# Levicoz/Options-model

Measured on AMD Instinct MI355X. Metric: paths x steps / sec (whole American pricing: path-gen + LSM + mean), higher is better.
Workload: dtype f32

## Files before the change

### options_model_amd/csrc/omc_api.hip

```cpp
#include <sched.h>

#include <algorithm>

#include "omc_ctx.h"

namespace omc::abi {

thread_local std::string g_err;
size_t g_alloc_limit = 0;

int check_market(double S0, double K, double T, double r)
{
    if (!(S0 > 0) || !(K > 0) || !(T > 0)) return fail(-1, "S0, K, T must be positive.");
    if (!(r >= 0)) return fail(-2, "r must be non-negative.");
    return 0;
}

int check_sizes(int64_t n_paths, int n_steps)
{
    if (n_paths <= 0 || n_steps <= 0)
        return fail(-3, "num_simulations and num_time_steps must be positive integers.");
    if (n_steps > omc::kMaxSteps) return fail(-8, "num_time_steps exceeds the supported maximum (4094).");
    return 0;
}
// ... 689 lines not shown
    int rc = bind_in(c);
    if (rc) return rc;
    if (!bytes) return 0;
    HIP_TRY(hipMemcpyAsync(dst, src, bytes, kind, c->stream));
    HIP_TRY(hipStreamSynchronize(c->stream));
    return 0;
}

int omc_memcpy_h2d(omc_ctx* c, void* dst, const void* src, size_t bytes)
{
    return copy_and_wait(c, dst, src, bytes, hipMemcpyHostToDevice);
}

int omc_memcpy_d2h(omc_ctx* c, void* dst, const void* src, size_t bytes)
{
    return copy_and_wait(c, dst, src, bytes, hipMemcpyDeviceToHost);
}

int omc_set_option(omc_ctx* c, const char* key, int64_t value)
{
    if (!c || !key) return fail(-7, "null pointer.");
    if (!strcmp(key, "gbm_vec")) c->gbm_vec = (int)value;
    else if (!strcmp(key, "alloc_limit")) g_alloc_limit = value > 0 ? (size_t)value : 0;
    else if (!strcmp(key, "fold_antithetic")) c->fold = value <= 0 ? 0 : (value >= 2 ? 2 : 1);
    else if (!strcmp(key, "pass2_tables")) c->pass2_tables = value ? 1 : 0;
    else if (!strcmp(key, "pass2_tables_irregular_every")) c->pass2_irr_every = value > 0 ? (int)value : 0;
    else if (!strcmp(key, "heston_vec")) c->heston_vec = (int)value;
    else if (!strcmp(key, "world_size")) c->world = value > 0 ? (int)value : 1;
    else if (!strcmp(key, "step_graph")) c->step_graph = value < 0 ? -1 : (value ? 1 : 0);
    else if (!strcmp(key, "seq_overlap")) c->seq_overlap = value < 0 ? -1 : (value ? 1 : 0);
    else if (!strcmp(key, "seq_event_stride")) c->seq_event_stride = value > 0 ? (int)value : 0;
    else if (!strcmp(key, "seq_step_k")) c->seq_step_k = value < 0 ? -1 : (int)(value > 32 ? 32 : value);
    else if (!strcmp(key, "seq_two_pass_k")) c->seq_two_pass_k = value < 0 ? -1 : (int)(value > 32 ? 32 : value);
    else if (!strcmp(key, "bounds_exercise_every")) {
        if (value < 0 || value > 2147483647) return fail(-4, "bounds_exercise_every must be in 0 .. 2^31 - 1.");
        c->bounds_every = value;
    }
    else if (!strcmp(key, "bounds_control_variate")) {
        if (value != 0 && value != 1) return fail(-4, "bounds_control_variate must be 0 or 1.");
        c->bounds_cv = (int)value;
    }
    else if (!strcmp(key, "bounds_cv_form")) {
        if (value != 0 && value != 1) return fail(-4, "bounds_cv_form must be 0 or 1.");
        c->bounds_cv_form = (int)value;
    }
    else if (!strcmp(key, "chain_fused")) c->chain_fused = value ? 1 : 0;
    else if (!strcmp(key, "chain_k")) c->chain_k = value < 1 ? -1 : (int)(value > 16 ? 16 : value);
    else if (!strcmp(key, "seq_step_wgs")) c->seq_step_wgs = value > 0 ? (int)value : 0;
    else if (!strcmp(key, "p2p_exchange")) c->p2p_use = value ? 1 : 0;
    else if (!strcmp(key, "p2p_deadline_ms") || !strcmp(key, "p2p_first_deadline_ms")) {
        if (value <= 0) return fail(-4, "a p2p deadline must be positive.");
        (key[4] == 'f' ? c->p2p_first_deadline_s : c->p2p_deadline_s) = (double)value * 1e-3;
        if (c->p2p) omc::p2p_set_deadline(c->p2p, c->p2p_deadline_s, c->p2p_first_deadline_s);
    }
    else return fail(-4, "unknown option key.");
    return 0;
}

int omc_set_allreduce_hook(omc_ctx* c, omc_allreduce_fn fn, void* user)
{
    if (!c) return fail(-7, "null context.");
    if (fn) {
        int rc;
        if ((rc = bind(c))) return rc;
        if ((rc = c->seq_vote.ensure(kVoteBytes))) return rc;
    }
// ... 128 lines not shown
```

### options_model_amd/csrc/omc_api_seq.hip

```cpp
#include <cstdlib>

#include "omc_ctx.h"

using namespace omc::abi;

extern "C" {

static int pricing_events(omc_ctx* c, int i, hipEvent_t** out)
{
    const int k = c->seq_event_stride, s = i == 0 ? 0 : (k > 0 && i % k == 0) ? i / k : -1;
    *out = s == 0 ? c->ev : nullptr;
    if (s <= 0) return 0;
    while (c->ev_pool.size() < 7 * (size_t)s) {
        hipEvent_t e = nullptr;
        HIP_TRY(hipEventCreate(&e));
        c->ev_pool.push_back(e);
    }
    *out = c->ev_pool.data() + 7 * (size_t)(s - 1);
    return 0;
}

static bool seq_overlap_enabled(const omc_ctx* c)
{
    if (c->seq_overlap >= 0) return c->seq_overlap != 0;
// ... 248 lines not shown
        }
        if (i0 == 0 && p2p) omc::p2p_begin_call(c->p2p);
        if (i0 == 0) HIP_TRY(hipEventRecord(c->ev[0], c->stream));
        for (int k = 0; k < Kb; ++k)
            if ((rc = enqueue_paths(c, &p[i0 + k], (float*)((char*)c->mS.p + sbytes * (size_t)k), ld))) return rc;
        if (i0 == 0) HIP_TRY(hipEventRecord(c->ev[1], c->stream));
        for (int t = N; t >= 1; --t) {
            HIP_TRY(omc::lsm_step_multi(c->stream, c->mtable.p, Kb, G, sem, vec4, N, t));
            if (ext && t >= 2) {
                if (p2p) {
                    HIP_TRY(omc::p2p_exchange_step_multi(c->p2p, c->stream, Kb, t - 1));
                    c->p2p_used = true;
                } else {
                    HIP_TRY(omc::lsm_reduce_step_moments_multi(c->stream, c->mtable.p, Kb, t - 1));
                    if ((rc = allreduce(c, gmomK + (size_t)(t - 1) * 8 * (size_t)Kb, 8 * Kb))) return rc;
                }
            }
        }
        HIP_TRY(omc::lsm_final_multi(c->stream, c->mtable.p, Kb, M));
        if (i0 == 0) HIP_TRY(hipEventRecord(c->ev[2], c->stream));
    }
    return 0;
}

int omc_seq_step_width(omc_ctx* c, const omc_params* p, int n)
{
    if (!c || !p || n <= 0) return 0;
    for (int i = 0; i < n; ++i)
        if (check_params(&p[i])) return 0;
    return seq_multi_width(c, p, n);
}


static bool seq_group_eligible(const omc_ctx* c, const omc_params* q)
{
    return c->pass2_tables && q->semantics == OMC_SEM_TWO_PASS && q->n_steps >= 2 && fold_applies(c, q);
}

static int seq_group_run(const omc_ctx* c, const omc_params* p, int n)
{
    if (c->distributed() || !seq_group_eligible(c, &p[0])) return 1;
    double c0, g;
    omc::gbm_fold_constants(p[0].S0, p[0].K, p[0].r, p[0].sigma, p[0].T, p[0].n_steps, &c0, &g);
    int run = 1;
    for (; run < n; ++run) {
        const omc_params& q = p[run];
        if (!seq_group_eligible(c, &q) || q.n_paths != p[0].n_paths || q.n_steps != p[0].n_steps || q.r != p[0].r ||
            q.T != p[0].T)
            break;
        double c0q, gq;
        omc::gbm_fold_constants(q.S0, q.K, q.r, q.sigma, q.T, q.n_steps, &c0q, &gq);
        if (c0q != c0 || gq != g) break;
    }
    return run;
}

static size_t seq_group_matrix_bytes(const omc_params* p)
{
    return sizeof(float) * (size_t)padded_ld(p->n_paths / 2) * ((size_t)p->n_steps + 1);
}

static int seq_group_ideal(const omc_ctx* c, const omc_params* p, int run)
{
    if (run < 2) return 1;
    static const int env_k = getenv("OMC_SEQ_TWO_PASS_K") ? atoi(getenv("OMC_SEQ_TWO_PASS_K")) : -1;
    int k = c->seq_two_pass_k >= 0 ? c->seq_two_pass_k : env_k;
    if (k < 0) k = (double)p[0].n_paths * (double)p[0].n_steps > 536870912.0 ? 1 : 8;
    if (k > omc::kSeqGroupMax) k = omc::kSeqGroupMax;
    if (k > run) k = run;
    return k < 2 ? 1 : k;
}

static int seq_group_fit(const omc_ctx* c, const omc_params* p, int k)
{
    const GroupLayout L(p[0].n_paths, p[0].n_steps);
    const int fit = (int)(seq_resident_budget(c, c->gS.cap + c->gstate.cap) / ((double)seq_group_matrix_bytes(p) + (double)L.per));
    if (k > fit) k = fit;
    return k < 2 ? 1 : k;
}

static int seq_group_reserve(omc_ctx* c, const omc_params* p, int run, int* K_out)
{
    *K_out = 1;
    int K = seq_group_ideal(c, p, run);
    const GroupLayout L(p[0].n_paths, p[0].n_steps);
    const size_t sbytes = seq_group_matrix_bytes(p);
    if (K >= 2 && (c->gS.cap < sbytes * (size_t)K || c->gstate.cap < L.per * (size_t)K)) K = seq_group_fit(c, p, K);
    while (K >= 2) {
        int rc = c->gS.ensure(sbytes * (size_t)K);
        if (!rc) rc = c->gstate.ensure(L.per * (size_t)K);
        if (!rc) break;
        if (rc != (int)hipErrorOutOfMemory && rc != (int)hipErrorMemoryAllocation) return rc;
        K /= 2;
    }
    *K_out = K < 2 ? 1 : K;
    return 0;
}

static int enqueue_seq_group(omc_ctx* c, const omc_params* p, int i0, int Kb, double* dst)
{
    int rc;
    const int64_t M = p[i0].n_paths;
    const int N = p[i0].n_steps;
    const size_t sbytes = seq_group_matrix_bytes(&p[i0]);
    int64_t ld = 0;
    const double* cK = nullptr;
    if ((rc = plan_storage(c, &p[i0], 0, &ld, &cK))) return rc;
    omc::LsmWorkspace w0;
    if ((rc = prepare_lsm(c, M, N, p[i0].r, p[i0].T, true, false, &w0))) return rc;
    if (!cK || ld != padded_ld(M / 2) || Kb > omc::kSeqGroupMax) return fail(-4, "a grouped two-pass sequence needs folded storage.");
    TwoPassGroup grp(GroupLayout(M, N), c->gstate.p, w0, true);
    hipEvent_t* evs[omc::kSeqGroupMax];
    for (int k = 0; k < Kb; ++k) {
        hipEvent_t* grown = nullptr;
        if ((rc = pricing_events(c, i0 + k, &grown))) return rc;
    }
    for (int k = 0; k < Kb; ++k) {
        const omc_params& q = p[i0 + k];
        float* S = (float*)((char*)c->gS.p + sbytes * (size_t)k);
        omc::LsmProblem prob{S, ld, M, N, q.is_put ? 1 : 0, q.K, q.r, q.T};
        prob.fold_cK = cK;
        grp.add(prob, dst + 8 * (size_t)(i0 + k));
        if ((rc = pricing_events(c, i0 + k, &evs[k]))) return rc;
        if (evs[k]) {
            grp.w[k].ev_p1_end = evs[k][4]; grp.w[k].ev_p2_end = evs[k][6];
            HIP_TRY(hipEventRecord(evs[k][0], c->stream));
        }
        if ((rc = enqueue_paths(c, &q, S, ld, true))) return rc;
        if (evs[k]) HIP_TRY(hipEventRecord(evs[k][1], c->stream));
        HIP_TRY(omc::lsm_pass1_sweep(c->stream, prob, grp.w[k], &grp.g.ntiles));
    }
    HIP_TRY(grp.reduce_pass1(c->stream));
    HIP_TRY(grp.build_tables(c->stream));
    for (int k = 0; k < Kb; ++k) {
        if (evs[k]) HIP_TRY(hipEventRecord(evs[k][5], c->stream));
        HIP_TRY(omc::lsm_pass2_sweep(c->stream, grp.prob[k], grp.w[k], false, true, &grp.g.nblk));
    }
    HIP_TRY(grp.finalize(c->stream));
    if (i0 == 0) HIP_TRY(hipEventRecord(c->ev[2], c->stream));
    return 0;
}

int omc_seq_group_width(omc_ctx* c, const omc_params* p, int n)
{
    if (!c || !p || n <= 0) return 0;
    for (int i = 0; i < n; ++i)
        if (check_params(&p[i])) return 0;
    const int run = seq_group_run(c, p, n);
    const int k = seq_group_ideal(c, p, run);
    return k < 2 ? 1 : seq_group_fit(c, p, k);
}

int omc_price_american_seq(omc_ctx* c, const omc_params* p, int n, omc_result* res)
{
    int rc;
    if ((rc = bind(c))) return rc;
    if (!p || !res || n <= 0) return fail(-7, "null pointer or empty sequence.");
    for (int i = 0; i < n; ++i)
        if ((rc = check_params(&p[i]))) return rc;
    if (!c->hres_dev) {
        for (int i = 0; i < n; ++i)
            if ((rc = omc_price_american(c, &p[i], &res[i], nullptr, 0))) return rc;
        return 0;
    }
    if (c->seq_cap < n) {
        if (c->seq_pin) (void)hipHostFree(c->seq_pin);
        c->seq_pin = c->seq_dev = nullptr;
        c->seq_cap = 0;
        HIP_TRY(hipHostMalloc((void**)&c->seq_pin, sizeof(double) * 8 * (size_t)n, hipHostMallocMapped));
        HIP_TRY(hipHostGetDevicePointer((void**)&c->seq_dev, c->seq_pin, 0));
        c->seq_cap = n;
    }
    hipEvent_t ev_end = c->ev[2];
    if (!c->ev_seq) HIP_TRY(hipEventCreate(&c->ev_seq));
    ev_end = c->ev_seq;
    const bool overlapped = seq_can_overlap(c, p, n);
    int multi = 1;
    if (!overlapped && (rc = seq_multi_reserve(c, p, n, &multi))) return rc;
    if (overlapped && (rc = enqueue_seq_overlapped(c, p, n, c->seq_pin))) return rc;
    const bool dist = c->distributed() && !overlapped;
    if (dist && (rc = c->seq_local.ensure(sizeof(double) * 8 * (size_t)n))) return rc;
    double* local = (double*)c->seq_local.p;
    c->defer_result_allreduce = dist;
    if (multi > 1 && (rc = enqueue_seq_step_multi(c, p, n, multi, dist ? local : c->seq_dev))) {
        c->defer_result_allreduce = false;
        return rc;
    }
    for (int i = 0; i < n && !overlapped && multi <= 1;) {
        int run = seq_group_run(c, &p[i], n - i), Kg = 1;
        if (run >= 2 && (rc = seq_group_reserve(c, &p[i], run, &Kg))) break;
        while (Kg >= 2 && run >= 2 && !rc) {
            const int Kb = Kg < run ? Kg : run;
            rc = enqueue_seq_group(c, p, i, Kb, c->seq_dev);
            i += Kb;
            run -= Kb;
        }
        for (; run >= 1 && !rc; ++i, --run) {
            hipEvent_t* evs = nullptr;
            if ((rc = pricing_events(c, i, &evs))) break;
            rc = enqueue_pricing(c, &p[i], nullptr, 0, dist ? local + 8 * (size_t)i : c->seq_dev + 8 * (size_t)i,
                                 evs, nullptr);
            if (!rc && evs && i == 0 && hipEventRecord(evs[2], c->stream) != hipSuccess) rc = fail(999, "hipEventRecord failed");
        }
        if (rc) break;
    }
    c->defer_result_allreduce = false;
    if (rc) return rc;
    if (dist) {
        if (c->p2p_used) HIP_TRY(omc::p2p_stamp_results(c->p2p, c->stream, local, n));
        if ((rc = allreduce(c, local, 8 * n))) return rc;
        HIP_TRY(hipMemcpyAsync(c->seq_pin, local, sizeof(double) * 8 * (size_t)n, hipMemcpyDeviceToHost, c->stream));
    }
    HIP_TRY(hipEventRecord(ev_end, c->stream));
    if ((rc = wait_stream(c))) return rc;
    if ((rc = check_p2p(c, c->seq_pin, n))) return rc;
    float ms_all = 0;
    HIP_TRY(hipEventElapsedTime(&ms_all, c->ev[0], ev_end));
    omc_result timed;
    memset(&timed, 0, sizeof timed);
    for (int i = 0; i < n; ++i) {
        hipEvent_t* evs = nullptr;
        if ((multi <= 1 || i == 0) && (rc = pricing_events(c, i, &evs))) return rc;
        if (evs) {
            if ((rc = read_kernel_times(evs, &p[i], &timed, i == 0))) return rc;
            if (multi > 1) timed.ms_paths /= (double)multi;
        }
        fill_result(&res[i], c->seq_pin + 8 * (size_t)i, c->distributed() ? p[i].n_paths * c->world : p[i].n_paths,
                    c->distributed() ? c->world : 1);
        res[i].ms_paths = timed.ms_paths;
// ... 12 lines not shown
```

### options_model_amd/csrc/omc_ctx.h

```cpp
#pragma once
#include <hip/hip_runtime.h>

#include <cmath>
#include <cstdio>
#include <cstring>
#include <functional>
#include <string>
#include <vector>

#include "../../include/omc.h"
#include "omc_basket.h"
#include "omc_bounds.h"
#include "omc_comm.h"
#include "omc_kernels.h"
#include "omc_p2p.h"

namespace omc::abi {

extern thread_local std::string g_err;

inline int fail(int code, const char* msg)
{
    g_err = msg;
    return code;
}

#define HIP_TRY(expr)                                                                      \
    do {                                                                                   \
        hipError_t e_ = (expr);                                                            \
        if (e_ != hipSuccess) {                                                            \
            char buf_[256];                                                                \
            snprintf(buf_, sizeof buf_, "%s failed: %s (%s:%d)", #expr, hipGetErrorString(e_), \
                     __FILE__, __LINE__);                                                  \
            g_err = buf_;                                                                  \
            return (int)e_ > 0 ? (int)e_ : 999;                                            \
        }                                                                                  \
    } while (0)

extern size_t g_alloc_limit;
// ... 106 lines not shown
    std::function<hipError_t(hipStream_t, int64_t i0, int64_t ni)> inner;
    std::function<hipError_t(hipStream_t, const omc::BoundsSched& sc, int64_t i0, int64_t ni)> inner_sched;
    std::function<hipError_t(hipStream_t, double* result)> lower_cv;
    std::function<hipError_t(hipStream_t, int64_t i0, int64_t ni)> inner_cv;
    std::function<hipError_t(hipStream_t, const omc::BoundsSched& sc, int64_t i0, int64_t ni)> inner_sched_cv;
    double cv_e0 = 0.0;
    std::function<int(const omc::LsmWorkspace& w, float* S, int64_t ld)> own_policy;
    std::function<hipError_t(hipStream_t, double* result)> walk;
    std::function<hipError_t(hipStream_t, double* betas_out)> read_policy;
};
int run_bounds(omc_ctx* c, const omc_params* p, const omc_bounds_config* cfg, const double* betas, double* betas_out,
               double* q_out, double* samples_out, omc_bounds* out, const BoundsFlow& f);

struct GroupLayout {
    size_t o_gmom, o_betas, o_crit, o_part, per;
    GroupLayout(int64_t M, int N);
};
struct TwoPassGroup {
    TwoPassGroup(const GroupLayout& L, void* state, const omc::LsmWorkspace& w0, bool tables);
    void add(const omc::LsmProblem& p, double* result);
    hipError_t reduce_pass1(hipStream_t st) const { return omc::lsm_group_reduce_pass1(st, g, K); }
    hipError_t build_tables(hipStream_t st) const { return omc::lsm_group_crit_build(st, g, K); }
    hipError_t finalize(hipStream_t st) const { return omc::lsm_group_finalize(st, g, K); }
    int K = 0;
    omc::LsmProblem prob[omc::kSeqGroupMax];
    omc::LsmWorkspace w[omc::kSeqGroupMax];
    omc::SeqGroupArgs g = {};

private:
    GroupLayout L;
    char* state;
    omc::LsmWorkspace w0;
    bool tables;
};

}

using omc::abi::DevBuf;

struct RowsCache {
    bool valid = false;
    const float* S = nullptr;
    int64_t ld = 0, M = 0;
    int N = 0, is_put = 0;
    double K = 0, r = 0, T = 0;
    int64_t R = 0;
    double st[16] = {0};
};

constexpr size_t kVoteBytes = 1024;

struct omc_ctx {
    int device = 0;
    hipStream_t stream = nullptr;
    bool own_stream = false;
    DevBuf S, sx, tex, ex, D, part, gmom, betas, part1, result, scratch, sweep_args, crit;
    DevBuf bslab, btable, bres, bdisc;
    DevBuf mlp_part, mlp_loss, mlp_wt;
    DevBuf mlp_gred, shard;
    DevBuf cn_scratch, cn_data, cn_net, cn_cont;
    std::vector<char> h_table;
    std::vector<double> h_disc, h_bres;
    std::vector<double> hD;
    int D_N = -1;
    double D_r = 0, D_T = 0;
    const double* D_ptr = nullptr;
    double hres[8];
    double* hres_pin = nullptr;
    double* hres_dev = nullptr;
    double *seq_pin = nullptr, *seq_dev = nullptr;
    int seq_cap = 0;
    hipEvent_t ev_seq = nullptr;
    hipEvent_t ev_entry = nullptr;
    hipEvent_t ev[7] = {nullptr, nullptr, nullptr, nullptr, nullptr, nullptr, nullptr};
    std::vector<hipEvent_t> ev_pool;
    int seq_event_stride = 0;
    DevBuf mS, mstate, mtable;
    DevBuf mb_slab, mb_table, mb_bc;
    std::vector<double> mb_bc_host;
    double mb_beta1 = -1.0, mb_beta2 = -1.0;
    size_t mb_bc_cap = 0;
    char* mtab_pin = nullptr;
    int mtab_slot = 0;
    int seq_step_k = -1;
    int seq_step_wgs = 0;
    DevBuf gS, gstate;
    int seq_two_pass_k = -1;
    int gbm_vec = 0, heston_vec = 0;
    int fold = 1;
    int pass2_tables = 1;
    int pass2_irr_every = 0;
    DevBuf foldC;
    DevBuf gk_part, gk_res;
    DevBuf bar_part, bar_res;
    DevBuf div_tab;
    int64_t bounds_every = 0;
    int bounds_cv = 0;
    int bounds_cv_form = 0;
    DevBuf bnd;
    DevBuf chain_fold;
    DevBuf chain_sched;
    int chain_fused = 0;
    int chain_k = -1;
    struct FoldKey { int N = -1; double c0 = 0, g = 0; } fold_key[2];
    int world = 1;
    omc_allreduce_fn hook = nullptr;
    void* hook_user = nullptr;
    omc::Comm* comm = nullptr;
    omc::P2P* p2p = nullptr;
    int p2p_use = 1;
    bool p2p_used = false;
    double p2p_deadline_s = 2.0;
    double p2p_first_deadline_s = 30.0;
    hipStream_t comm_stream = nullptr;
    hipEvent_t ev_moments[2] = {nullptr, nullptr}, ev_reduced[2] = {nullptr, nullptr};
    RowsCache rows_cache;
    DevBuf S2, seq_local, part1b, gmomb, seq_vote;
    int seq_overlap = -1;
    bool defer_result_allreduce = false;
    hipGraph_t sweep_graph = nullptr;
// ... 14 lines not shown
```

### options_model_amd/csrc/omc_kernels.h

```cpp
#pragma once
#include <hip/hip_runtime.h>
#include <stdint.h>

#include <atomic>
#include <cmath>

#include "omc_dispatch.h"

namespace omc {

inline hipError_t set_max_dynamic_lds(std::atomic<uint64_t>& mask, const void* kernel, size_t bytes)
{
    int dev = 0;
    hipError_t e = hipGetDevice(&dev);
    if (e != hipSuccess) return e;
    const uint64_t bit = 1ull << (dev & 63);
    if (mask.load(std::memory_order_acquire) & bit) return hipSuccess;
    e = hipFuncSetAttribute(kernel, hipFuncAttributeMaxDynamicSharedMemorySize, (int)bytes);
    if (e != hipSuccess) return e;
    mask.fetch_or(bit, std::memory_order_release);
    return hipSuccess;
}

struct PathSpec {
// ... 123 lines not shown
    });
}
size_t lsm_sweep_args_bytes();
void lsm_sweep_args_image(const LsmProblem& p, const LsmWorkspace& w, int semantics, bool fill_state, void* out,
                          bool external_moments = false);
int lsm_multi_groups(int64_t M, int K, int device_cus);
hipError_t lsm_step_multi(hipStream_t st, const void* table_dev, int K, int G, int semantics, bool vec4, int N, int t);
hipError_t lsm_reduce_step_moments_multi(hipStream_t st, const void* table_dev, int K, int t);
hipError_t lsm_final_multi(hipStream_t st, const void* table_dev, int K, int64_t M);
hipError_t lsm_sweep_indirect(hipStream_t st, const LsmProblem& p, const LsmWorkspace& w, int semantics,
                              const void* args_dev);

hipError_t lsm_pass1_moments(hipStream_t st, const LsmProblem& p, const LsmWorkspace& w);
hipError_t lsm_pass2_apply(hipStream_t st, const LsmProblem& p, const LsmWorkspace& w,
                           bool write_state, bool solve_from_moments = false);
hipError_t lsm_pass1_sweep(hipStream_t st, const LsmProblem& p, const LsmWorkspace& w, int64_t* ntiles);
hipError_t lsm_reduce_pass1(hipStream_t st, const LsmWorkspace& w, int64_t ntiles, int N);
bool lsm_pass2_tables(const LsmProblem& p, const LsmWorkspace& w, bool write_state);
hipError_t lsm_pass2_sweep(hipStream_t st, const LsmProblem& p, const LsmWorkspace& w, bool write_state,
                           bool solve_from_moments, int* nblk);
constexpr int kPass1Tpw = 4, kFoldTpw = 2;
struct Pass1Geometry {
    bool v4 = false;
    int tchunk = 32;
    int64_t ntiles = 0;
    dim3 grid;
};
Pass1Geometry lsm_pass1_geometry(const LsmProblem& p);
struct FoldGeometry {
    Pass1Geometry p1;
    int fvec = 2, vec2 = 1, nblk = 0;
};
FoldGeometry lsm_fold_geometry(const LsmProblem& p);
constexpr int kSeqGroupMax = 32;
struct SeqGroupSlot {
    const double* part1;
    double* gmom;
    double* betas;
    uint32_t* crit;
    const double* part;
    double* result;
    const double* cK;
    double K, invK;
    int is_put;
    int N;
};
struct SeqGroupArgs {
    SeqGroupSlot slot[kSeqGroupMax];
    int64_t ntiles;
    int N, nblk;
    int irr_every, pad_;
};
static_assert(sizeof(SeqGroupSlot) == 80 && sizeof(SeqGroupArgs) == 80 * kSeqGroupMax + 24 && sizeof(SeqGroupArgs) <= 4096,
              "the group's argument block travels by value in the kernel arguments");
SeqGroupSlot lsm_group_slot(const LsmProblem& p, const LsmWorkspace& w);
hipError_t lsm_group_reduce_pass1(hipStream_t st, const SeqGroupArgs& g, int K);
hipError_t lsm_group_crit_build(hipStream_t st, const SeqGroupArgs& g, int K);
hipError_t lsm_group_finalize(hipStream_t st, const SeqGroupArgs& g, int K);
hipError_t lsm_solve_betas(hipStream_t st, const double* gmom, double* betas, int N);
struct CritArgs {
    const double* gmom = nullptr;
    const double* betas = nullptr;
    double* betas_out = nullptr;
    const double* cK = nullptr;
    uint32_t* tab = nullptr;
    int N = 0, is_put = 0;
// ... 114 lines not shown
```

### options_model_amd/csrc/omc_lsm.hip

```cpp
#include "omc_lsm_dev.h"

#include <cstdlib>
#include <cstring>

namespace omc {

template <int SEM, int VEC, int BLOCK>
__global__ __launch_bounds__(BLOCK) void lsm_step_kernel(StepArgs a)
{
    lsm_step_body<SEM, VEC, BLOCK>(a, blockIdx.x, a.nblk);
}

template <int SEM, int VEC, int BLOCK>
__global__ __launch_bounds__(BLOCK) void lsm_step_ind_kernel(const StepArgs* __restrict__ ap, int t)
{
    StepArgs a = *ap;
    a.t = t;
    lsm_step_body<SEM, VEC, BLOCK>(a, blockIdx.x, a.nblk);
}

__global__ __launch_bounds__(kBlock) void lsm_reduce_step_kernel(const double* part, double* gmom, int t,
                                                                 int nblk, int pstride, int gstride)
{
    lsm_reduce_step_body(part, gmom, t, nblk, pstride, gstride);
}

template <int VEC, int TPW, int PUT>
__global__ __launch_bounds__(kBlock) void lsm_pass1_kernel(Pass1Args a) { lsm_pass1_body<VEC, TPW, PUT>(a); }

__global__ __launch_bounds__(kBlock) void lsm_reduce_pass1_kernel(const double* part1, double* gmom,
                                                                  int64_t ntiles, int N)
{
    lsm_reduce_pass1_body(part1, gmom, ntiles, N);
}

__global__ void lsm_solve_betas_kernel(const double* __restrict__ gmom, double* __restrict__ betas, int N)
{
    lsm_solve_all_body(gmom, betas, N);
}

template <int VEC, bool WRITE_STATE>
__global__ __launch_bounds__(kBlock) void lsm_pass2_kernel(Pass2Args a) { lsm_pass2_body<VEC, WRITE_STATE>(a); }

template <int VEC, int TPW, int PUT>
__global__ __launch_bounds__(kBlock) void lsm_pass1_fold_kernel(Pass1Args a) { lsm_pass1_fold_body<VEC, TPW, PUT>(a); }
template <int VEC, int PUT, bool TAB>
__global__ __launch_bounds__(kBlock) void lsm_pass2_fold_kernel(Pass2Args a) { lsm_pass2_fold_body<VEC, PUT, TAB>(a); }

__global__ __launch_bounds__(128) void lsm_crit_build_kernel(CritArgs a) { lsm_crit_build_body(a); }
__global__ __launch_bounds__(kBlock) void lsm_crit_check_kernel(const uint32_t* tab, const double* betas, const double* cK,
                                                                int N, int is_put, double K, double invK,
                                                                unsigned long long* mism)
{
    lsm_crit_check_body(tab, betas, cK, N, is_put, K, invK, mism);
}

__global__ void lsm_fold_table_kernel(double* __restrict__ cK, int N, double c0, double g)
{
    if (threadIdx.x == 0 && blockIdx.x == 0) fold_table_fill(cK, N, c0, g);
}

template <int VEC>
__global__ __launch_bounds__(kBlock) void lsm_final_kernel(FinalArgs a) { lsm_final_body<VEC>(a); }

template <int VEC>
__global__ __launch_bounds__(kBlock) void lsm_final_ind_kernel(const FinalArgs* __restrict__ ap)
{
    lsm_final_body<VEC>(*ap);
}

__global__ __launch_bounds__(kBlock) void lsm_finalize_kernel(const double* part, const double* gmom,
                                                              double* result, int nblk, int N, int pstride)
{
    lsm_finalize_body(part, gmom, result, nblk, N, pstride);
}

struct FinalizeArgs {
    const double* part;
    const double* gmom;
    double* result;
// ... 337 lines not shown
    const int nblk = fold ? geo.nblk : lsm_step_blocks(p.M);
    *nblk_out = nblk;
    if (fold && write_state) return hipErrorInvalidValue;
    Pass2Args a = pass2_args(p, w, nblk);
    const bool tab = lsm_pass2_tables(p, w, write_state);
    if (tab) {
        a.crit = w.crit;
    } else if (solve_from_moments) {
        a.gmom = w.gmom;
        a.betas_out = w.betas;
    }
    const size_t dyn = sizeof(double) * 4 * (size_t)(p.N + 1);
    const dim3 grid(nblk), block(kBlock);
    if (fold) {
        for_vec(geo.vec2, [&](auto vec) {
            for_put(p.is_put, [&](auto put) {
                for_flag(tab, [&](auto tb) {
                    constexpr int VEC = decltype(vec)::value, PUT = decltype(put)::value;
                    hipLaunchKernelGGL((lsm_pass2_fold_kernel<VEC, PUT, decltype(tb)::value>), grid, block, dyn, st, a);
                });
            });
        });
    } else {
        for_vec4(rows_aligned(4, p.M, p.S, p.ld), [&](auto vec) {
            for_flag(write_state, [&](auto ws) {
                hipLaunchKernelGGL((lsm_pass2_kernel<decltype(vec)::value, decltype(ws)::value>), grid, block, dyn, st, a);
            });
        });
    }
    if (w.ev_p2_end) (void)hipEventRecord(w.ev_p2_end, st);
    return hipGetLastError();
}

hipError_t lsm_pass2_apply(hipStream_t st, const LsmProblem& p, const LsmWorkspace& w,
                           bool write_state, bool solve_from_moments)
{
    if (w.ev_p2_begin) (void)hipEventRecord(w.ev_p2_begin, st);
    const bool tab = lsm_pass2_tables(p, w, write_state);
    if (tab) {
        CritArgs c;
        c.gmom = solve_from_moments ? w.gmom : nullptr; c.betas = w.betas; c.betas_out = solve_from_moments ? w.betas : nullptr;
        c.cK = p.fold_cK; c.tab = w.crit;
        c.N = p.N; c.is_put = p.is_put; c.K = p.K; c.irr_every = w.crit_irr_every;
        const hipError_t e = lsm_crit_build(st, c);
        if (e != hipSuccess) return e;
    }
    int nblk = 0;
    const hipError_t e = lsm_pass2_sweep(st, p, w, write_state, solve_from_moments, &nblk);
    return e != hipSuccess ? e : lsm_finalize(st, w.part, w.gmom, w.result, nblk, p.N);
}

SeqGroupSlot lsm_group_slot(const LsmProblem& p, const LsmWorkspace& w)
{
    SeqGroupSlot s;
    s.part1 = w.part1; s.gmom = w.gmom; s.betas = w.betas; s.crit = w.crit; s.part = w.part; s.result = w.result;
    s.cK = p.fold_cK;
    s.K = p.K; s.invK = 1.0 / p.K; s.is_put = p.is_put; s.N = p.N;
    return s;
}

hipError_t lsm_group_reduce_pass1(hipStream_t st, const SeqGroupArgs& g, int K)
{
    if (g.N < 2) return hipSuccess;
    hipLaunchKernelGGL(lsm_reduce_pass1_group_kernel, dim3(g.N - 1, K), dim3(kBlock), 0, st, g);
    return hipGetLastError();
}
// ... 59 lines not shown
```

### options_model_amd/csrc/omc_lsm_dev.h

```cpp
#pragma once
#include "omc_device.h"
#include "omc_kernels.h"
#include "omc_crit.h"
#include <type_traits>

namespace omc {


constexpr int kPStride = kMaxLsmBlocks;

template <int VEC>
__device__ __forceinline__ void loadf(const float* __restrict__ p, float (&v)[VEC])
{
    if constexpr (VEC == 4) {
        const float4 x = *reinterpret_cast<const float4*>(p);
        v[0] = x.x; v[1] = x.y; v[2] = x.z; v[3] = x.w;
    } else if constexpr (VEC == 2) {
        const float2 x = *reinterpret_cast<const float2*>(p);
        v[0] = x.x; v[1] = x.y;
    } else {
        static_assert(VEC == 1, "loadf: 1, 2 or 4 floats");
        v[0] = *p;
    }
}
// ... 447 lines not shown
                load_rows(bufB, min(t + 4, tl));
                __builtin_amdgcn_sched_barrier(0);
                process(put_tag, bufC, t + 2);
            }
        }
    };
    if (PUT == 1 || (PUT < 0 && is_put))
        sweep(std::true_type{});
    else
        sweep(std::false_type{});
}

__device__ __forceinline__ double fold_rcp(float s)
{
    const double x = (double)s;
    double r = __builtin_amdgcn_rcp(x);
    r = fma(fma(-x, r, 1.0), r, r);
    return r;
}
__device__ __forceinline__ double fold_u_rcp(double cK_t, double rcp_s) { return fma(cK_t, rcp_s, -1.0); }
__device__ __forceinline__ double fold_u(double cK_t, float s) { return fold_u_rcp(cK_t, fold_rcp(s)); }
__device__ __forceinline__ double fold_pay(double u, double K, int is_put) { return is_put ? -K * u : K * u; }
__device__ __forceinline__ void fold_table_fill(double* __restrict__ tab, int N, double c0, double g)
{
    double c = c0;
    tab[0] = c;
    for (int t = 1; t <= N; ++t) {
        c *= g;
        tab[t] = c;
    }
}
constexpr int kFoldMaxChunk = 64;

template <int VEC, int TPW, int PUT = -1>
__device__ __forceinline__ void lsm_pass1_fold_body(Pass1Args a)
{
    __shared__ double wl[kBlock / 64][kWaveRedDoubles];
    __shared__ double shD[kBlock / 64][kFoldMaxChunk];
    __shared__ double shC[kBlock / 64][kFoldMaxChunk];
    const int lane = threadIdx.x & 63, wave = threadIdx.x >> 6;
    const int64_t tg = (int64_t)xcd_block((int)blockIdx.x, (int)gridDim.x) * (kBlock / 64) + wave;
    if (tg >= a.ntiles) return;
    const int64_t base = tg * (64 * VEC * TPW) + (int64_t)lane * VEC;
    const int t0 = 1 + ((int)gridDim.y - 1 - (int)blockIdx.y) * a.tchunk;
    const int t1 = min(t0 + a.tchunk, a.N);
    if (t0 >= t1) return;
    const double K = a.K, invK = a.invK;
    const int is_put = PUT < 0 ? a.is_put : PUT;
    for (int i = lane; i < t1 - t0; i += 64) {
        shD[wave][i] = a.D[a.N - (t0 + i)];
        shC[wave][i] = a.cK[t0 + i];
    }
    const float* colp[TPW];
    double pNA[TPW][VEC], pNB[TPW][VEC];
    bool valid[TPW];
    const double cKN = a.cK[a.N];
    float sn[TPW][VEC];
#pragma unroll
    for (int k = 0; k < TPW; ++k) {
        const int64_t j = base + (int64_t)k * 64 * VEC;
        valid[k] = j < a.M;
        colp[k] = a.S + (valid[k] ? j : 0);
        loadf<VEC>(colp[k] + (int64_t)a.N * a.ld, sn[k]);
    }
    auto load_rows = [&](float (&buf)[TPW][VEC], int t) {
#pragma unroll
        for (int k = 0; k < TPW; ++k) loadf_stream<VEC>(colp[k] + (int64_t)t * a.ld, buf[k]);
    };
    float bufA[TPW][VEC], bufB[TPW][VEC], bufC[TPW][VEC];
    const int tl = t1 - 1;
    load_rows(bufA, t0);
    load_rows(bufB, min(t0 + 1, tl));
    __builtin_amdgcn_sched_barrier(0);
#pragma unroll
    for (int k = 0; k < TPW; ++k) {
#pragma unroll
        for (int v = 0; v < VEC; ++v) {
// ... 130 lines not shown
    bo[0] = beta[0]; bo[1] = beta[1]; bo[2] = beta[2]; bo[3] = m[0];
}


struct Fit {
    double b0, b1, b2;
};
__device__ __forceinline__ Fit no_fit() { return {__builtin_huge_val(), 0.0, 0.0}; }

__device__ __forceinline__ Fit fit_given(const double* __restrict__ betas, int t, int N)
{
    if (t >= 1 && t < N && betas[(size_t)t * 4 + 3] > 0.5)
        return {betas[(size_t)t * 4], betas[(size_t)t * 4 + 1], betas[(size_t)t * 4 + 2]};
    return no_fit();
}

__device__ __forceinline__ Fit fit_solved(const double* __restrict__ gmom, int t, int N, double* betas_out)
{
    const bool inner = t >= 1 && t < N;
    double m[8], beta[3] = {0.0, 0.0, 0.0};
#pragma unroll
    for (int q = 0; q < 8; ++q) m[q] = inner ? gmom[(size_t)t * 8 + q] : 0.0;
    if (inner) solve_poly2(m, beta);
    if (inner && betas_out) {
        double* bo = betas_out + (size_t)t * 4;
        bo[0] = beta[0]; bo[1] = beta[1]; bo[2] = beta[2]; bo[3] = m[0];
    }
    if (inner && m[0] > 0.5) return {beta[0], beta[1], beta[2]};
    return no_fit();
}

template <bool FOLD>
__device__ __forceinline__ void fits_to_lds(double* sh_b, const double* __restrict__ gmom, double* betas_out,
                                            const double* __restrict__ betas, const double* __restrict__ cK, int N)
{
    auto put = [&](int t, const Fit& f) {
        sh_b[4 * t] = f.b0;
        sh_b[4 * t + 1] = f.b1;
        sh_b[4 * t + 2] = f.b2;
        sh_b[4 * t + 3] = FOLD ? cK[t] : 0.0;
    };
    if (gmom) {
        for (int t = threadIdx.x; t <= N; t += kBlock) put(t, fit_solved(gmom, t, N, blockIdx.x == 0 ? betas_out : nullptr));
    } else {
        for (int t = threadIdx.x; t <= N; t += kBlock) put(t, fit_given(betas, t, N));
    }
    __syncthreads();
}
__device__ __forceinline__ Fit fit_lds(const double* sh_b, int t) { return {sh_b[4 * t], sh_b[4 * t + 1], sh_b[4 * t + 2]}; }

struct PayU {
    double imm, u;
};
__device__ __forceinline__ PayU pay_stored(double s, double K, double invK, int is_put)
{
    return {is_put ? K - s : s - K, fma(s, invK, -1.0)};
}
__device__ __forceinline__ PayU pay_partner(double ck, float s, double K, int is_put)
{
    const double u = fold_u(ck, s);
    return {fold_pay(u, K, is_put), u};
}
__device__ __forceinline__ bool exercises(const PayU& p, const Fit& f)
{
    return (p.imm > 0.0) & (p.imm > fma(p.u, fma(p.u, f.b2, f.b1), f.b0));
}

__device__ __forceinline__ bool crit_in(uint4 iv, uint32_t b) { return crit_in(iv.x, iv.y, iv.z, iv.w, b); }

__device__ __forceinline__ double add_cash_flow(double* acc, double imm, double D, bool exercised)
{
    const double cf = (imm > 0.0 ? imm : 0.0) * D;
    acc[0] += cf;
    acc[1] += cf * cf;
    acc[2] += exercised ? 1.0 : 0.0;
    acc[3] += cf == 0.0 ? 1.0 : 0.0;
// ... 188 lines not shown
        auto live = [&]() {
            bool l = false;
#pragma unroll
            for (int v = 0; v < VEC; ++v) l |= (tex[v] == N);
            return l;
        };
        constexpr int U = 8;
        int t = N - 1;
        const float* col = a.S + j;
        for (; t >= U && live(); t -= U) {
            float st[U][VEC];
#pragma unroll
            for (int k = 0; k < U; ++k) loadf_stream<VEC>(col + (int64_t)(t - k) * a.ld, st[k]);
#pragma unroll
            for (int k = 0; k < U; ++k) decide(st[k], t - k);
        }
        for (; t >= 1 && live(); --t) {
            float st[VEC];
            loadf_stream<VEC>(col + (int64_t)t * a.ld, st);
            decide(st, t);
        }
#pragma unroll
        for (int v = 0; v < VEC; ++v) add_cash_flow(acc, payoff_d(sx[v], K, is_put), a.D[tex[v] - 1], tex[v] < N);
        if (WRITE_STATE) {
            storef<VEC>(a.sx + j, sx);
            storei<VEC>(a.tex + j, tex);
        }
    }
    const double s = block_reduce8(acc, red);
    if (tid < 64 && (tid & 7) == 0) a.part[(size_t)(tid >> 3) * a.pstride + blockIdx.x] = s;
}

template <int VEC, int PUT = -1, bool TAB = false>
__device__ __forceinline__ void lsm_pass2_fold_body(Pass2Args a)
{
    if ((int)blockIdx.x >= a.nblk) return;
    __shared__ double red[kNQ * kRedStride];
    extern __shared__ double sh_b[];
    uint32_t* sh_t = reinterpret_cast<uint32_t*>(sh_b);
    const int tid = threadIdx.x;
    const int N = a.N;
    bool irr_any = false;
    if (TAB) irr_any = crit_load_tables(a.crit, sh_t, N);
    else fits_to_lds<true>(sh_b, a.gmom, a.betas_out, a.betas, a.cK, N);
    const double K = a.K, invK = a.invK;
    const int is_put = PUT < 0 ? a.is_put : PUT;
    double acc[8];
#pragma unroll
    for (int q = 0; q < 8; ++q) acc[q] = 0.0;
    const int64_t stride = (int64_t)a.nblk * kBlock * VEC;
    auto sweep = [&](auto chk) {
    constexpr bool CHK = decltype(chk)::value;
    for (int64_t j = ((int64_t)blockIdx.x * kBlock + tid) * VEC; j < a.M; j += stride) {
        float sxa[VEC], sxb[VEC];
        int32_t texa[VEC], texb[VEC];
        loadf<VEC>(a.S + (int64_t)N * a.ld + j, sxa);
#pragma unroll
        for (int v = 0; v < VEC; ++v) {
            sxb[v] = sxa[v];
            texa[v] = texb[v] = N;
        }
        auto decide_f64 = [&](const float (&row)[VEC], int t, const Fit& f, double ck) {
#pragma unroll
            for (int v = 0; v < VEC; ++v) {
                const bool ex = (texa[v] == N) & exercises(pay_stored(row[v], K, invK, is_put), f);
                sxa[v] = ex ? row[v] : sxa[v];
                texa[v] = ex ? t : texa[v];
                const bool exb = (texb[v] == N) & exercises(pay_partner(ck, row[v], K, is_put), f);
                sxb[v] = exb ? row[v] : sxb[v];
                texb[v] = exb ? t : texb[v];
            }
        };
        auto decide = [&](const float (&row)[VEC], int t) {
            if constexpr (!TAB) {
                decide_f64(row, t, fit_lds(sh_b, t), sh_b[4 * t + 3]);
            } else {
                const uint4 ta = *reinterpret_cast<const uint4*>(sh_t + 8 * t);
                if (CHK && __builtin_amdgcn_readfirstlane(ta.x) == kCritIrregular) {
                    decide_f64(row, t, fit_given(a.betas, t, N), a.cK[t]);
                    return;
                }
                const uint4 tb = *reinterpret_cast<const uint4*>(sh_t + 8 * t + 4);
#pragma unroll
                for (int v = 0; v < VEC; ++v) {
                    const uint32_t bits = __float_as_uint(row[v]);
                    const bool ex = (texa[v] == N) & crit_in(ta, bits);
                    sxa[v] = ex ? row[v] : sxa[v];
                    texa[v] = ex ? t : texa[v];
                    const bool exb = (texb[v] == N) & crit_in(tb, bits);
                    sxb[v] = exb ? row[v] : sxb[v];
                    texb[v] = exb ? t : texb[v];
                }
            }
        };
        auto live = [&]() {
            bool l = false;
#pragma unroll
            for (int v = 0; v < VEC; ++v) l |= (texa[v] == N) | (texb[v] == N);
            return l;
        };
        walk_rows<VEC, TAB>(a.S + j, a.ld, N, decide, live);
#pragma unroll
        for (int v = 0; v < VEC; ++v) {
            add_cash_flow(acc, payoff_d(sxa[v], K, is_put), a.D[texa[v] - 1], texa[v] < N);
            const double ck = TAB ? a.cK[texb[v]] : sh_b[4 * texb[v] + 3];
            add_cash_flow(acc, pay_partner(ck, sxb[v], K, is_put).imm, a.D[texb[v] - 1], texb[v] < N);
        }
    }
    };
    if (TAB && irr_any) sweep(std::true_type{});
    else sweep(std::false_type{});
    const double s = block_reduce8(acc, red);
    if (tid < 64 && (tid & 7) == 0) a.part[(size_t)(tid >> 3) * a.pstride + blockIdx.x] = s;
}

struct FinalArgs {
    float* sx;
    int32_t* tex;
    const float* live;
    int64_t M;
    int N, is_put, tval, fill_state;
    double K;
    const double* D;
    double* part;
    int nblk, pstride;
};

template <int VEC>
__device__ __forceinline__ void lsm_final_body(FinalArgs a)
{
    if ((int)blockIdx.x >= a.nblk) return;
    __shared__ double red[kNQ * kRedStride];
    const int tid = threadIdx.x;
    double acc[8];
#pragma unroll
    for (int q = 0; q < 8; ++q) acc[q] = 0.0;
    const int64_t stride = (int64_t)a.nblk * kBlock * VEC;
    for (int64_t j = ((int64_t)blockIdx.x * kBlock + tid) * VEC; j < a.M; j += stride) {
        float sx[VEC];
        int32_t tex[VEC];
        loadf<VEC>(a.sx + j, sx);
        loadi<VEC>(a.tex + j, tex);
        if (a.live) {
            float sn[VEC];
            loadf<VEC>(a.live + j, sn);
            bool any = false;
// ... 43 lines not shown
```

Baseline: 799.3 billion.

## Defer grouped pass-2 sweeps and fuse them with the next group's pass-1

For grouped two-pass American pricing sequences, the pass-2 sweeps of one group are deferred and run inside a combined kernel that also executes the next group's pass-1 sweep, with the two blocks sharing LDS through a union. This uses double-buffered path and state storage (gS2/gstate2), and is enabled by default when the folded column count is small. The aim is to fill the GPU with concurrent independent work and to cut launch and tail overhead between dependent small kernels. The cost is a second buffer set, heavier scheduling logic, and possible LDS or occupancy pressure in the fused kernel.

```diff
diff --git a/options_model_amd/csrc/omc_api.hip b/options_model_amd/csrc/omc_api.hip
--- a/options_model_amd/csrc/omc_api.hip
+++ b/options_model_amd/csrc/omc_api.hip
@@ -745,6 +745,9 @@
     else if (!strcmp(key, "seq_event_stride")) c->seq_event_stride = value > 0 ? (int)value : 0;
     else if (!strcmp(key, "seq_step_k")) c->seq_step_k = value < 0 ? -1 : (int)(value > 32 ? 32 : value);
     else if (!strcmp(key, "seq_two_pass_k")) c->seq_two_pass_k = value < 0 ? -1 : (int)(value > 32 ? 32 : value);
+    else if (!strcmp(key, "seq_defer_pass2")) c->seq_defer_pass2 = value < 0 ? -1 : (value ? 1 : 0);
+    else if (!strcmp(key, "seq_defer_q")) c->seq_defer_q = value < 1 ? -1 : (int)(value > 8 ? 8 : value);
+    else if (!strcmp(key, "seq_defer_order")) c->seq_defer_order = value < 0 ? -1 : (value ? 1 : 0);
     else if (!strcmp(key, "bounds_exercise_every")) {
         if (value < 0 || value > 2147483647) return fail(-4, "bounds_exercise_every must be in 0 .. 2^31 - 1.");
         c->bounds_every = value;
diff --git a/options_model_amd/csrc/omc_api_seq.hip b/options_model_amd/csrc/omc_api_seq.hip
--- a/options_model_amd/csrc/omc_api_seq.hip
+++ b/options_model_amd/csrc/omc_api_seq.hip
@@ -304,6 +304,10 @@
 }
 
 
+constexpr int64_t kSeqDeferMaxColumns = int64_t(1) << 18;
+constexpr int kSeqDeferQ = 1;
+constexpr bool kSeqDeferPass1First = false;
+
 static bool seq_group_eligible(const omc_ctx* c, const omc_params* q)
 {
     return c->pass2_tables && q->semantics == OMC_SEM_TWO_PASS && q->n_steps >= 2 && fold_applies(c, q);
@@ -351,9 +355,21 @@
     return k < 2 ? 1 : k;
 }
 
-static int seq_group_reserve(omc_ctx* c, const omc_params* p, int run, int* K_out)
+static bool seq_defer_enabled(const omc_ctx* c, const omc_params* p)
+{
+    if (c->seq_defer_pass2 >= 0) return c->seq_defer_pass2 != 0;
+    static const int env = [] {
+        const char* e = getenv("OMC_SEQ_DEFER_PASS2");
+        return e ? atoi(e) : -1;
+    }();
+    if (env >= 0) return env != 0;
+    return p->n_paths / 2 <= kSeqDeferMaxColumns;
+}
+
+static int seq_group_reserve(omc_ctx* c, const omc_params* p, int run, int* K_out, bool* second)
 {
     *K_out = 1;
+    *second = false;
     int K = seq_group_ideal(c, p, run);
     const GroupLayout L(p[0].n_paths, p[0].n_steps);
     const size_t sbytes = seq_group_matrix_bytes(p);
@@ -366,10 +382,36 @@
         K /= 2;
     }
     *K_out = K < 2 ? 1 : K;
-    return 0;
-}
-
-static int enqueue_seq_group(omc_ctx* c, const omc_params* p, int i0, int Kb, double* dst)
+    if (K < 2 || run <= K || !seq_defer_enabled(c, p)) return 0;
+    const size_t needS = sbytes * (size_t)K, needT = L.per * (size_t)K;
+    if (c->gS2.cap < needS || c->gstate2.cap < needT) {
+        if (g_alloc_limit && 2 * needS > g_alloc_limit) return 0;
+        if (seq_resident_budget(c, c->gS2.cap + c->gstate2.cap) < (double)needS + (double)needT) return 0;
+        int rc = c->gS2.ensure(needS);
+        if (!rc) rc = c->gstate2.ensure(needT);
+        if (rc == (int)hipErrorOutOfMemory || rc == (int)hipErrorMemoryAllocation) return 0;
+        if (rc) return rc;
+    }
+    *second = true;
+    return 0;
+}
+
+static int seq_flush_pending(omc_ctx* c, SeqPending* pend, const bool* done = nullptr)
+{
+    if (!pend->active()) return 0;
+    TwoPassGroup& g = *pend->grp;
+    std::unique_ptr<TwoPassGroup> keep = std::move(pend->grp);
+    for (int k = 0; k < g.K; ++k) {
+        if (done && done[k]) continue;
+        if (pend->ev_p2_begin[k]) HIP_TRY(hipEventRecord(pend->ev_p2_begin[k], c->stream));
+        HIP_TRY(omc::lsm_pass2_sweep(c->stream, g.prob[k], g.w[k], false, true, &g.g.nblk));
+    }
+    HIP_TRY(g.finalize(c->stream));
+    if (pend->first) HIP_TRY(hipEventRecord(c->ev[2], c->stream));
+    return 0;
+}
+
+static int enqueue_seq_group(omc_ctx* c, const omc_params* p, int i0, int Kb, double* dst, SeqPending* pend, bool defer)
 {
     int rc;
     const int64_t M = p[i0].n_paths;
@@ -381,15 +423,27 @@
     omc::LsmWorkspace w0;
     if ((rc = prepare_lsm(c, M, N, p[i0].r, p[i0].T, true, false, &w0))) return rc;
     if (!cK || ld != padded_ld(M / 2) || Kb > omc::kSeqGroupMax) return fail(-4, "a grouped two-pass sequence needs folded storage.");
-    TwoPassGroup grp(GroupLayout(M, N), c->gstate.p, w0, true);
+    const int set = pend->active() ? 1 - pend->set : 0;
+    char* Sset = (char*)(set ? c->gS2.p : c->gS.p);
+    std::unique_ptr<TwoPassGroup> own(new TwoPassGroup(GroupLayout(M, N), set ? c->gstate2.p : c->gstate.p, w0, true));
+    TwoPassGroup& grp = *own;
+    {
+        omc::LsmProblem probe{(const float*)Sset, ld, M, N, 1, p[i0].K, p[i0].r, p[i0].T};
+        probe.fold_cK = cK;
+        const omc::FoldGeometry fg = omc::lsm_fold_geometry(probe);
+        if (!fg.p1.v4 || fg.vec2 != 2) defer = false;
+    }
     hipEvent_t* evs[omc::kSeqGroupMax];
+    bool done[omc::kSeqGroupMax] = {};
+    const int vq = c->seq_defer_q > 0 ? c->seq_defer_q : kSeqDeferQ;
+    const bool p1_first = c->seq_defer_order >= 0 ? c->seq_defer_order != 0 : kSeqDeferPass1First;
     for (int k = 0; k < Kb; ++k) {
         hipEvent_t* grown = nullptr;
         if ((rc = pricing_events(c, i0 + k, &grown))) return rc;
     }
     for (int k = 0; k < Kb; ++k) {
         const omc_params& q = p[i0 + k];
-        float* S = (float*)((char*)c->gS.p + sbytes * (size_t)k);
+        float* S = (float*)(Sset + sbytes * (size_t)k);
         omc::LsmProblem prob{S, ld, M, N, q.is_put ? 1 : 0, q.K, q.r, q.T};
         prob.fold_cK = cK;
         grp.add(prob, dst + 8 * (size_t)(i0 + k));
@@ -400,17 +454,23 @@
         }
         if ((rc = enqueue_paths(c, &q, S, ld, true))) return rc;
         if (evs[k]) HIP_TRY(hipEventRecord(evs[k][1], c->stream));
-        HIP_TRY(omc::lsm_pass1_sweep(c->stream, prob, grp.w[k], &grp.g.ntiles));
-    }
+        if (pend->active() && k < pend->grp->K && !pend->ev_p2_begin[k] &&
+            omc::lsm_pass1_pass2_fusable(prob, grp.w[k], pend->grp->prob[k], pend->grp->w[k])) {
+            HIP_TRY(omc::lsm_pass1_pass2_sweep(c->stream, prob, grp.w[k], pend->grp->prob[k], pend->grp->w[k], vq, p1_first,
+                                               &grp.g.ntiles, &pend->grp->g.nblk));
+            done[k] = true;
+        } else {
+            HIP_TRY(omc::lsm_pass1_sweep(c->stream, prob, grp.w[k], &grp.g.ntiles));
+        }
+    }
+    if ((rc = seq_flush_pending(c, pend, done))) return rc;
     HIP_TRY(grp.reduce_pass1(c->stream));
     HIP_TRY(grp.build_tables(c->stream));
-    for (int k = 0; k < Kb; ++k) {
-        if (evs[k]) HIP_TRY(hipEventRecord(evs[k][5], c->stream));
-        HIP_TRY(omc::lsm_pass2_sweep(c->stream, grp.prob[k], grp.w[k], false, true, &grp.g.nblk));
-    }
-    HIP_TRY(grp.finalize(c->stream));
-    if (i0 == 0) HIP_TRY(hipEventRecord(c->ev[2], c->stream));
-    return 0;
+    pend->grp = std::move(own);
+    pend->set = set;
+    pend->first = i0 == 0;
+    for (int k = 0; k < Kb; ++k) pend->ev_p2_begin[k] = evs[k] ? evs[k][5] : nullptr;
+    return defer ? 0 : seq_flush_pending(c, pend);
 }
 
 int omc_seq_group_width(omc_ctx* c, const omc_params* p, int n)
@@ -460,13 +520,17 @@
     }
     for (int i = 0; i < n && !overlapped && multi <= 1;) {
         int run = seq_group_run(c, &p[i], n - i), Kg = 1;
-        if (run >= 2 && (rc = seq_group_reserve(c, &p[i], run, &Kg))) break;
+        bool defer = false;
+        if (run >= 2 && (rc = seq_group_reserve(c, &p[i], run, &Kg, &defer))) break;
+        SeqPending pend;
         while (Kg >= 2 && run >= 2 && !rc) {
             const int Kb = Kg < run ? Kg : run;
-            rc = enqueue_seq_group(c, p, i, Kb, c->seq_dev);
+            rc = enqueue_seq_group(c, p, i, Kb, c->seq_dev, &pend, defer);
             i += Kb;
             run -= Kb;
         }
+        if (rc) (void)seq_flush_pending(c, &pend);
+        else rc = seq_flush_pending(c, &pend);
         for (; run >= 1 && !rc; ++i, --run) {
             hipEvent_t* evs = nullptr;
             if ((rc = pricing_events(c, i, &evs))) break;
diff --git a/options_model_amd/csrc/omc_ctx.h b/options_model_amd/csrc/omc_ctx.h
--- a/options_model_amd/csrc/omc_ctx.h
+++ b/options_model_amd/csrc/omc_ctx.h
@@ -5,6 +5,7 @@
 #include <cstdio>
 #include <cstring>
 #include <functional>
+#include <memory>
 #include <string>
 #include <vector>
 
@@ -177,6 +178,14 @@
     char* state;
     omc::LsmWorkspace w0;
     bool tables;
+};
+
+struct SeqPending {
+    std::unique_ptr<TwoPassGroup> grp;
+    hipEvent_t ev_p2_begin[omc::kSeqGroupMax] = {};
+    bool first = false;
+    int set = 0;
+    bool active() const { return grp != nullptr; }
 };
 
 }
@@ -231,6 +240,10 @@
     int seq_step_wgs = 0;
     DevBuf gS, gstate;
     int seq_two_pass_k = -1;
+    DevBuf gS2, gstate2;
+    int seq_defer_pass2 = -1;
+    int seq_defer_q = -1;
+    int seq_defer_order = -1;
     int gbm_vec = 0, heston_vec = 0;
     int fold = 1;
     int pass2_tables = 1;
diff --git a/options_model_amd/csrc/omc_kernels.h b/options_model_amd/csrc/omc_kernels.h
--- a/options_model_amd/csrc/omc_kernels.h
+++ b/options_model_amd/csrc/omc_kernels.h
@@ -179,6 +179,9 @@
     int fvec = 2, vec2 = 1, nblk = 0;
 };
 FoldGeometry lsm_fold_geometry(const LsmProblem& p);
+bool lsm_pass1_pass2_fusable(const LsmProblem& pB, const LsmWorkspace& wB, const LsmProblem& pA, const LsmWorkspace& wA);
+hipError_t lsm_pass1_pass2_sweep(hipStream_t st, const LsmProblem& pB, const LsmWorkspace& wB, const LsmProblem& pA,
+                                 const LsmWorkspace& wA, int q, bool pass1_first, int64_t* ntiles, int* nblk);
 constexpr int kSeqGroupMax = 32;
 struct SeqGroupSlot {
     const double* part1;
diff --git a/options_model_amd/csrc/omc_lsm.hip b/options_model_amd/csrc/omc_lsm.hip
--- a/options_model_amd/csrc/omc_lsm.hip
+++ b/options_model_amd/csrc/omc_lsm.hip
@@ -43,9 +43,43 @@
 __global__ __launch_bounds__(kBlock) void lsm_pass2_kernel(Pass2Args a) { lsm_pass2_body<VEC, WRITE_STATE>(a); }
 
 template <int VEC, int TPW, int PUT>
-__global__ __launch_bounds__(kBlock) void lsm_pass1_fold_kernel(Pass1Args a) { lsm_pass1_fold_body<VEC, TPW, PUT>(a); }
+__global__ __launch_bounds__(kBlock) void lsm_pass1_fold_kernel(Pass1Args a)
+{
+    __shared__ Pass1FoldLds sh;
+    lsm_pass1_fold_body<VEC, TPW, PUT>(a, sweep_geom(), sh);
+}
 template <int VEC, int PUT, bool TAB>
-__global__ __launch_bounds__(kBlock) void lsm_pass2_fold_kernel(Pass2Args a) { lsm_pass2_fold_body<VEC, PUT, TAB>(a); }
+__global__ __launch_bounds__(kBlock) void lsm_pass2_fold_kernel(Pass2Args a)
+{
+    __shared__ Pass2FoldLds sh;
+    lsm_pass2_fold_body<VEC, PUT, TAB>(a, sweep_geom(), sh);
+}
+
+struct FusedWork {
+    int p2_phys, p1_first, p1_row, p1_gx, p1_gy, p1_lead;
+};
+template <int VEC1, int PUT1, int VEC2, int PUT2>
+__global__ __launch_bounds__(kBlock) void lsm_pass1_pass2_fold_kernel(Pass1Args a1, Pass2Args a2, FusedWork w)
+{
+    __shared__ union Lds {
+        Pass1FoldLds p1;
+        Pass2FoldLds p2;
+    } sh;
+    const int b = (int)blockIdx.x;
+    const int n1 = w.p1_row * w.p1_gy;
+    const int b1 = w.p1_lead ? b : b - w.p1_first, b2 = w.p1_lead ? b - n1 : b;
+    if (b2 >= 0 && b2 < w.p2_phys) {
+        for (int v = b2; v < a2.nblk; v += w.p2_phys) {
+            if (v != b2) __syncthreads();
+            lsm_pass2_fold_body<VEC2, PUT2, true>(a2, SweepGeom{(unsigned)v, 0u, (unsigned)a2.nblk, 1u}, sh.p2);
+        }
+        return;
+    }
+    if (b1 < 0 || b1 >= n1) return;
+    const int by = b1 / w.p1_row, bx = b1 - by * w.p1_row;
+    if (bx >= w.p1_gx) return;
+    lsm_pass1_fold_body<VEC1, kFoldTpw, PUT1>(a1, SweepGeom{(unsigned)bx, (unsigned)by, (unsigned)w.p1_gx, (unsigned)w.p1_gy}, sh.p1);
+}
 
 __global__ __launch_bounds__(128) void lsm_crit_build_kernel(CritArgs a) { lsm_crit_build_body(a); }
 __global__ __launch_bounds__(kBlock) void lsm_crit_check_kernel(const uint32_t* tab, const double* betas, const double* cK,
@@ -449,6 +483,47 @@
     return hipGetLastError();
 }
 
+bool lsm_pass1_pass2_fusable(const LsmProblem& pB, const LsmWorkspace& wB, const LsmProblem& pA, const LsmWorkspace& wA)
+{
+    if (!pB.fold_cK || !pA.fold_cK || pB.N < 2 || !lsm_pass2_tables(pA, wA, false)) return false;
+    if (wB.ev_p1_begin || wB.ev_p1_end || wA.ev_p2_end) return false;
+    const FoldGeometry gB = lsm_fold_geometry(pB), gA = lsm_fold_geometry(pA);
+    if (!gB.p1.v4 || gA.vec2 != 2) return false;
+    const size_t lds = std::max(sizeof(Pass1FoldLds), sizeof(Pass2FoldLds)) + sizeof(double) * 4 * (size_t)(pA.N + 1);
+    return lds <= 64 * 1024;
+}
+
+hipError_t lsm_pass1_pass2_sweep(hipStream_t st, const LsmProblem& pB, const LsmWorkspace& wB, const LsmProblem& pA,
+                                 const LsmWorkspace& wA, int q, bool pass1_first, int64_t* ntiles, int* nblk)
+{
+    const Pass1Geometry g1 = lsm_fold_geometry(pB).p1;
+    const FoldGeometry gA = lsm_fold_geometry(pA);
+    const Pass1Args a1 = pass1_args(pB, wB, g1.ntiles, g1.tchunk);
+    Pass2Args a2 = pass2_args(pA, wA, gA.nblk);
+    a2.crit = wA.crit;
+    *ntiles = a1.ntiles;
+    *nblk = gA.nblk;
+    if (q < 1) q = 1;
+    FusedWork w;
+    w.p2_phys = (gA.nblk + q - 1) / q;
+    w.p1_first = (w.p2_phys + 7) / 8 * 8;
+    w.p1_gx = (int)g1.grid.x;
+    w.p1_gy = (int)g1.grid.y;
+    w.p1_row = (w.p1_gx + 7) / 8 * 8;
+    w.p1_lead = pass1_first ? 1 : 0;
+    const int64_t n1 = (int64_t)w.p1_row * w.p1_gy;
+    const int64_t blocks = pass1_first ? n1 + w.p2_phys : w.p1_first + n1;
+    if (blocks > INT32_MAX) return hipErrorInvalidValue;
+    const size_t dyn = sizeof(double) * 4 * (size_t)(pA.N + 1);
+    for_put(pB.is_put, [&](auto put1) {
+        for_put(pA.is_put, [&](auto put2) {
+            hipLaunchKernelGGL((lsm_pass1_pass2_fold_kernel<4, decltype(put1)::value, 2, decltype(put2)::value>),
+                               dim3((unsigned)blocks), dim3(kBlock), dyn, st, a1, a2, w);
+        });
+    });
+    return hipGetLastError();
+}
+
 hipError_t lsm_pass2_apply(hipStream_t st, const LsmProblem& p, const LsmWorkspace& w,
                            bool write_state, bool solve_from_moments)
 {
diff --git a/options_model_amd/csrc/omc_lsm_dev.h b/options_model_amd/csrc/omc_lsm_dev.h
--- a/options_model_amd/csrc/omc_lsm_dev.h
+++ b/options_model_amd/csrc/omc_lsm_dev.h
@@ -503,17 +503,33 @@
 }
 constexpr int kFoldMaxChunk = 64;
 
+struct SweepGeom {
+    unsigned bx, by, gx, gy;
+};
+__device__ __forceinline__ SweepGeom sweep_geom()
+{
+    return {blockIdx.x, blockIdx.y, gridDim.x, gridDim.y};
+}
+struct Pass1FoldLds {
+    double wl[kBlock / 64][kWaveRedDoubles];
+    double shC[kBlock / 64][kFoldMaxChunk];
+    double shD[kBlock / 64][kFoldMaxChunk];
+};
+struct Pass2FoldLds {
+    double red[kNQ * kRedStride];
+};
+
 template <int VEC, int TPW, int PUT = -1>
-__device__ __forceinline__ void lsm_pass1_fold_body(Pass1Args a)
-{
-    __shared__ double wl[kBlock / 64][kWaveRedDoubles];
-    __shared__ double shD[kBlock / 64][kFoldMaxChunk];
-    __shared__ double shC[kBlock / 64][kFoldMaxChunk];
+__device__ __forceinline__ void lsm_pass1_fold_body(Pass1Args a, const SweepGeom g, Pass1FoldLds& sh)
+{
+    auto& wl = sh.wl;
+    auto& shD = sh.shD;
+    auto& shC = sh.shC;
     const int lane = threadIdx.x & 63, wave = threadIdx.x >> 6;
-    const int64_t tg = (int64_t)xcd_block((int)blockIdx.x, (int)gridDim.x) * (kBlock / 64) + wave;
+    const int64_t tg = (int64_t)xcd_block((int)g.bx, (int)g.gx) * (kBlock / 64) + wave;
     if (tg >= a.ntiles) return;
     const int64_t base = tg * (64 * VEC * TPW) + (int64_t)lane * VEC;
-    const int t0 = 1 + ((int)gridDim.y - 1 - (int)blockIdx.y) * a.tchunk;
+    const int t0 = 1 + ((int)g.gy - 1 - (int)g.by) * a.tchunk;
     const int t1 = min(t0 + a.tchunk, a.N);
     if (t0 >= t1) return;
     const double K = a.K, invK = a.invK;
@@ -710,7 +726,8 @@
 
 template <bool FOLD>
 __device__ __forceinline__ void fits_to_lds(double* sh_b, const double* __restrict__ gmom, double* betas_out,
-                                            const double* __restrict__ betas, const double* __restrict__ cK, int N)
+                                            const double* __restrict__ betas, const double* __restrict__ cK, int N,
+                                            const unsigned bx = blockIdx.x)
 {
     auto put = [&](int t, const Fit& f) {
         sh_b[4 * t] = f.b0;
@@ -719,7 +736,7 @@
         sh_b[4 * t + 3] = FOLD ? cK[t] : 0.0;
     };
     if (gmom) {
-        for (int t = threadIdx.x; t <= N; t += kBlock) put(t, fit_solved(gmom, t, N, blockIdx.x == 0 ? betas_out : nullptr));
+        for (int t = threadIdx.x; t <= N; t += kBlock) put(t, fit_solved(gmom, t, N, bx == 0 ? betas_out : nullptr));
     } else {
         for (int t = threadIdx.x; t <= N; t += kBlock) put(t, fit_given(betas, t, N));
     }
@@ -974,17 +991,17 @@
 }
 
 template <int VEC, int PUT = -1, bool TAB = false>
-__device__ __forceinline__ void lsm_pass2_fold_body(Pass2Args a)
-{
-    if ((int)blockIdx.x >= a.nblk) return;
-    __shared__ double red[kNQ * kRedStride];
+__device__ __forceinline__ void lsm_pass2_fold_body(Pass2Args a, const SweepGeom g, Pass2FoldLds& sh)
+{
+    if ((int)g.bx >= a.nblk) return;
+    auto& red = sh.red;
     extern __shared__ double sh_b[];
     uint32_t* sh_t = reinterpret_cast<uint32_t*>(sh_b);
     const int tid = threadIdx.x;
     const int N = a.N;
     bool irr_any = false;
     if (TAB) irr_any = crit_load_tables(a.crit, sh_t, N);
-    else fits_to_lds<true>(sh_b, a.gmom, a.betas_out, a.betas, a.cK, N);
+    else fits_to_lds<true>(sh_b, a.gmom, a.betas_out, a.betas, a.cK, N, g.bx);
     const double K = a.K, invK = a.invK;
     const int is_put = PUT < 0 ? a.is_put : PUT;
     double acc[8];
@@ -993,7 +1010,7 @@
     const int64_t stride = (int64_t)a.nblk * kBlock * VEC;
     auto sweep = [&](auto chk) {
     constexpr bool CHK = decltype(chk)::value;
-    for (int64_t j = ((int64_t)blockIdx.x * kBlock + tid) * VEC; j < a.M; j += stride) {
+    for (int64_t j = ((int64_t)g.bx * kBlock + tid) * VEC; j < a.M; j += stride) {
         float sxa[VEC], sxb[VEC];
         int32_t texa[VEC], texb[VEC];
         loadf<VEC>(a.S + (int64_t)N * a.ld + j, sxa);
@@ -1053,7 +1070,7 @@
     if (TAB && irr_any) sweep(std::true_type{});
     else sweep(std::false_type{});
     const double s = block_reduce8(acc, red);
-    if (tid < 64 && (tid & 7) == 0) a.part[(size_t)(tid >> 3) * a.pstride + blockIdx.x] = s;
+    if (tid < 64 && (tid & 7) == 0) a.part[(size_t)(tid >> 3) * a.pstride + g.bx] = s;
 }
 
 struct FinalArgs {
```

New measurement: 791.2 billion. 0.99x the previous value.
